# eburhansjah/ec504_ImageEncoder

Hardware: AMD Instinct MI355X
Metric: 1080p I-frames/s (higher is better)
Workload: dtype f32 (colour fast path, FDCT: exact integers in floats) + f64 (colour ties) + int32 (VLC, packing); 1 GPU; 300 x 1920x1080 synthetic RGB frames per GPU, FULL region (all macroblocks), quality_factor 12, input and output resident in HBM; frames_per_gpu=300, global_frames=300, parallelism=frames sharded 300/GPU

## Files before the change

### ec504_imageencoder_amd/csrc/m1v_encode_tile_body.h

```cpp
    extern __shared__ __attribute__((aligned(16))) uint32_t lds[];
    const Geometry &g = a.g;
    const int tid = threadIdx.x;
    const int lane = tid & (kWave - 1);
    const int wave = __builtin_amdgcn_readfirstlane(tid >> 6);
    const bool chroma = wave == 2;
    constexpr int kStride = STAGE8 ? kStageStride8 : kStageStride16;

    uint32_t *vlc = lds + kTileVlc + wave * kVlcWords, *cnt = lds + kTileCnt, *G = lds + kTileG, *segtab = lds + kTileSegTab, *misc = lds + kTileMisc;
    const uint32_t lds0 = (uint32_t)(uintptr_t)(__attribute__((address_space(3))) uint32_t *)lds;
    const uint32_t region_off = (uint32_t)kTileFixedWords * 4u + (uint32_t)wave * a.luma_region;
    uint32_t *image = lds + kTileFixedWords + (2u * a.luma_region + a.chroma_region) / 4u;

    int frame, tile;
    frame_unit_of(blockIdx.x, a.n_frames, a.div_group, a.div_frame, frame, tile);
    const int tk = (int)udiv((uint32_t)tile, a.div_cols), tc = tile - tk * a.tile_cols;
    const int tr = (int)a.tile_row_order[tk];
    tile = tr * a.tile_cols + tc;
    int s0 = tc * kTileStrips, m0 = tr * kTileMbRows;
    const uint8_t *fbase;
    if constexpr (SURFACE) fbase = a.rgb + (unsigned long long)frame * frame_stride;
    else fbase = pixel_stage_rounds_down(a.rgb + (unsigned long long)frame * g.frame_bytes, s0, m0);
    const unsigned long long tile_index = (unsigned long long)frame * a.tiles_per_frame + tile;

    auto owner = [&](int ln, int &j, int &m, int &blk) {
        if (!chroma) {
            m = 2 * wave + (ln >> 5);
            blk = ((ln >> 4) & 1) * 2 + (ln & 1);
            j = (ln >> 1) & 7;
        } else {
            m = (ln >> 3) & 3;
            blk = 4 + (ln >> 5);
            j = ln & 7;
        }
    };
    const int strips_here = min(kTileStrips, g.n_strips - s0);
    int comp;
    {
        int j_, m_, blk_;
        owner(lane, j_, m_, blk_);
        comp = blk_ < 4 ? 0 : blk_ - 3;
    }

    TSTAMP_INIT();
    const uint32_t ring = lds0 + region_off;
    constexpr int kKeep = STAGE8 ? M1V_TILE_KEEP : M1V_TILE_KEEP_WIDE;
    RowStore<kKeep> rows;
    M1V_FRONT_HALF<R, kKeep, !SURFACE, BPP, SURFACE, ORDER>(
        g, fbase, ring, wave, lane, s0, m0, strips_here, comp,
        [&]() {
#pragma unroll
            for (int q = 0; q < kVlcWords / kWave; q++)
                dma4((uint32_t)lane * 4u, lds0 + (uint32_t)(kTileVlc + wave * kVlcWords + q * kWave) * 4u, a.tab->vlc + q * kWave);
        },
        [&]() {
            uint4 *image4 = reinterpret_cast<uint4 *>(image);
            for (int k = tid; k < (a.lds_words >> 2); k += kTileThreads) image4[k] = make_uint4(0u, 0u, 0u, 0u);
        },
        rows, row_pitch);
    const M1V_CONST_AS float *rq_t = reinterpret_cast<const M1V_CONST_AS float *>(reinterpret_cast<uintptr_t>(frame_rq_t(a.rq_all, a.qsel, frame)));
    int j, m, blk;
    {
        int ln = lane;
        asm volatile("" : "+v"(ln));
        owner(ln, j, m, blk);
    }
    const bool valid = j < strips_here && m0 + m < g.n_mbrows;
    const int e = j * kTileSegBlocks + m * 6 + blk;
    uint32_t *blkp = lds + region_off / 4u + lane * kStride;
    uint32_t lds_addr = (uint32_t)(uintptr_t)(__attribute__((address_space(3))) uint32_t *)blkp;
    TSTAMP(2);
    const int dc = columns_to_stage<STAGE8, kKeep>(rows, rq_t, lds_addr);
    const unsigned long long nz = (stage_nonzero_mask<STAGE8>(blkp, lds_addr) & ~1ull) | (dc != 0 ? 1ull : 0ull);
    TSTAMP(3);

    auto fetch = [&](int p) -> int { return fetch_level<STAGE8>(blkp, p); };
    uint32_t hdr = 0, bad = 0;
    int hlen = 0;
    BlockBits bb = {0, 0};
    dc_header(dc, blk < 4, blk, vlc, hdr, hlen);
    const unsigned long long emit = emit_set(nz);
    block_bits_pass1<STAGE8>(hdr, hlen, dc != 0, emit, vlc, fetch, bb.acc, bb.tot, bad);
    if (!valid) {
        bb.tot = 0;
        bad = 0;
    }
    cnt[e] = (uint32_t)bb.tot;
    TSTAMP(4);
    lds_barrier();
    TSTAMP(5);

    const uint32_t c0 = cnt[lane], c1 = cnt[64 + lane], c2 = cnt[128 + lane];
    const uint32_t i0 = wave_scan_inclusive(c0), i1 = wave_scan_inclusive(c1), i2 = wave_scan_inclusive(c2);
    const uint32_t t0 = (uint32_t)__builtin_amdgcn_readlane((int)i0, 63), t1 = (uint32_t)__builtin_amdgcn_readlane((int)i1, 63);
    G[lane] = i0 - c0;
    G[64 + lane] = t0 + i1 - c1;
    G[128 + lane] = t0 + t1 + i2 - c2;
    if (lane == 63) G[192] = t0 + t1 + i2;
    const uint32_t slice_bits = tr == 0 ? 38u : 0u;
    const uint32_t gs = G[min(lane, 8) * kTileSegBlocks];
    const uint32_t gs_next = (uint32_t)__builtin_amdgcn_update_dpp(0, (int)gs, 0x101, 0xf, 0xf, true);
    const uint32_t seg_bits = lane < strips_here ? slice_bits + (gs_next - gs) : 0u;
    const uint32_t seg_words = lane < 8 ? (seg_bits + 31u) >> 5 : 0u;
    const uint32_t seg_incl = row_scan_inclusive(seg_words);
    const uint32_t end_words = (uint32_t)__builtin_amdgcn_readlane((int)seg_incl, 7);
    if (lane < 8) {
        segtab[2 * lane] = gs;
        segtab[2 * lane + 1] = seg_incl - seg_words;
    }
    const uint32_t my_gs = segtab[2 * j], my_base = segtab[2 * j + 1];
    const uint32_t off = my_base * 32u + slice_bits + (G[e] - my_gs);
    TSTAMP(6);

    auto walk = [&](auto &sink) { walk_codes<STAGE8>(hdr, hlen, dc != 0, emit, vlc, fetch, sink); };
    unsigned long long *const strip_ctr_s0 = a.strip_ctr + ((unsigned long long)frame * (unsigned)g.n_strips + (unsigned)s0);
    auto strip_arrives = [&](uint32_t bits) -> unsigned long long {
#ifdef M1V_TILE_NOCOMPLETE
        __hip_atomic_fetch_add(strip_ctr_s0 + lane, (1ull << kCtrCountShift) | (unsigned long long)bits,
                               __ATOMIC_RELAXED, __HIP_MEMORY_SCOPE_AGENT);
        return 0ull;
#endif
        return atomicAdd(strip_ctr_s0 + lane, (1ull << kCtrCountShift) | (unsigned long long)bits);
    };
    auto strip_completes = [&](unsigned long long before, uint32_t bits) {
        if ((uint32_t)(before >> kCtrCountShift) == (uint32_t)a.tile_rows - 1u)
            atomicAdd(&a.frame_bytes[frame], ((before & kCtrBitsMask) + bits + 7ull) >> 3);
    };
    uint2 *seg_out = a.seg + (((unsigned long long)frame * (unsigned)a.tile_rows + (unsigned)tr) * (unsigned)g.n_strips + (unsigned)s0) + lane;
    auto slice_headers = [&](uint32_t *img, bool swapped) {
        if (tr == 0) {
            const uint32_t h0 = slice_word0(s0 + lane), h1 = kSliceWord1, w = seg_incl - seg_words;
            atomicOr(&img[w], swapped ? __builtin_bswap32(h0) : h0);
            atomicOr(&img[w + 1], swapped ? __builtin_bswap32(h1) : h1);
        }
    };

    if (end_words + 2 > (uint32_t)a.lds_words) {
        if (tid == 0) misc[0] = atomicAdd(a.arena_next, 1u);
        __syncthreads();
        const uint32_t got = misc[0];
        if (got >= a.arena_slots) {
            if (tid == 0) atomicOr(a.status, (uint32_t)M1V_STATUS_SCRATCH);
            if (wave == 0 && lane < strips_here) {
                *seg_out = make_uint2(0u, 0u);
                strip_completes(strip_arrives(0u), 0u);
            }
            return;
        }
        const unsigned long long where = a.arena_off + (unsigned long long)got * a.run_cap;
        uint32_t *big = reinterpret_cast<uint32_t *>(a.scratch + where);
        for (uint32_t i = tid; i < (a.run_cap >> 2); i += kTileThreads) big[i] = 0;
        __syncthreads();
        if (wave == 0 && lane < strips_here) {
            slice_headers(big, true);
            *seg_out = make_uint2(seg_bits, (uint32_t)(where >> 2) + (seg_incl - seg_words));
            strip_completes(strip_arrives(seg_bits), seg_bits);
        }
        if (valid) put_block<true>(big, off, bb, walk);
        if (bad) atomicOr(a.status, (uint32_t)M1V_STATUS_UNENCODABLE);
        return;
    }

    unsigned long long arrived = 0;
    if (wave == 0 && lane < strips_here) {
        slice_headers(image, false);
        *seg_out = make_uint2(seg_bits, (uint32_t)((tile_index * a.slot_bytes) >> 2) + (seg_incl - seg_words));
        arrived = strip_arrives(seg_bits);
    }
    if (valid) put_block<false>(image, off, bb, walk);
    TSTAMP(7);
    lds_barrier();
    TSTAMP(8);
    if (wave == 0 && lane < strips_here) strip_completes(arrived, seg_bits);
    uint32_t *slot32 = reinterpret_cast<uint32_t *>(a.scratch + tile_index * a.slot_bytes);
    for (uint32_t i = tid; i < end_words; i += kTileThreads) slot32[i] = __builtin_bswap32(image[i]);
    if (bad) atomicOr(a.status, (uint32_t)M1V_STATUS_UNENCODABLE);
    TSTAMP(9);
    TSTAMP_FLUSH();
```

### ec504_imageencoder_amd/csrc/m1v_kernels.hip

```cpp
#include <hip/hip_runtime.h>

#include <math.h>
#include <stdint.h>
#include <stdio.h>
#include <stdlib.h>
#include <string.h>

#include <type_traits>
#include <algorithm>
#include <vector>

#include "../../include/mpeg1_hip.h"

#define M1V_HD __host__ __device__ __forceinline__
#include "fdct_f32.h"

#pragma clang fp contract(off)

namespace {

constexpr int kWave = 64;
constexpr int kAcRows = 32;
constexpr int kVlcRowInfo = 0, kVlcEntries = 32, kVlcDcLuma = 144, kVlcDcChroma = 160, kVlcWords = 192;
constexpr int kMaxBlockBits = 886;
constexpr int kDefaultLdsWords = 4096;

__host__ __device__ constexpr int scan_pos(int k) {
    constexpr int t[64] = {0,  1,  5,  6,  14, 15, 27, 28, 2,  4,  7,  13, 16, 26, 29, 42,
                           3,  8,  12, 17, 25, 30, 41, 43, 9,  11, 18, 24, 31, 40, 44, 53,
                           10, 19, 23, 32, 39, 45, 52, 54, 20, 22, 33, 38, 46, 51, 55, 60,
                           21, 34, 37, 47, 50, 56, 59, 61, 35, 36, 48, 49, 57, 58, 62, 63};
    return t[k];
}
__host__ __device__ constexpr int scan_inv(int p) {
    for (int k = 0; k < 64; k++)
        if (scan_pos(k) == p) return k;
    return -1;
}

constexpr int kStageStride8 = 17, kStageStride16 = 33;
__host__ __device__ constexpr int stage_byte8(int p) { return ((p & 7) + 8 * (p >> 5)) * 4 + ((p >> 3) & 3); }
__host__ __device__ constexpr int stage_byte16(int p) { return ((p & 15) + 16 * (p >> 5)) * 4 + 2 * ((p >> 4) & 1); }

struct Tables {
    float rq[64];
    float rq_t[64];
    uint32_t vlc[kVlcWords];
    uint8_t hdr[256][44];
};

struct Geometry {
    int W, H, C;
    int n_strips, n_mbrows;
    int half_w;
    uint32_t strip_cap;
    unsigned long long frame_bytes;
};

#ifdef M1V_STAMPS
#define STAMP(ph)                                                                                  \
    do {                                                                                           \
        __builtin_amdgcn_sched_barrier(0);                                                         \
        unsigned long long now_ = __builtin_amdgcn_s_memtime();                                    \
        __builtin_amdgcn_s_waitcnt(0xC07F);                                                        \
        if ((threadIdx.x & 63) == 0) atomicAdd(&a.stamps[ph], now_ - stamp_t_);                    \
        stamp_t_ = __builtin_amdgcn_s_memtime();                                                   \
        __builtin_amdgcn_s_waitcnt(0xC07F);                                                        \
        __builtin_amdgcn_sched_barrier(0);                                                         \
    } while (0)
#define STAMP_INIT() unsigned long long stamp_t_ = __builtin_amdgcn_s_memtime(); __builtin_amdgcn_s_waitcnt(0xC07F)
#elif defined(M1V_MARKS)
#define STAMP(ph) asm volatile("; PHASE_MARK " #ph ::: "memory")
#define STAMP_INIT() asm volatile("; PHASE_MARK start" ::: "memory")
#else
#define STAMP(ph) do { } while (0)
#define STAMP_INIT() do { } while (0)
#endif

struct EncodeArgs {
    Geometry g;
    const uint8_t *rgb;
    const Tables *tab;
    const float *rq_all;
    const uint32_t *qsel;
    uint8_t *scratch;
    uint2 *seg;
    unsigned long long *strip_ctr;
    unsigned long long *frame_bytes;
    uint32_t *status;
    int n_frames;
    int threads;
    int lds_words;
    unsigned long long *stamps;
};


__device__ __forceinline__ int component_fp64(int r, int g, int b, double k0, double kr, double kg,
                                              double kb) {
    double acc = k0 + kr * (double)r;
    acc = acc + kg * (double)g;
    acc = acc + kb * (double)b;
    return (int)acc;
}

struct CompCoef {
    double k0, kr, kg, kb;
};
__device__ __forceinline__ CompCoef comp_coef(int comp) {
    CompCoef c;
    c.k0 = comp == 0 ? 0.0 : 128.0;
    c.kr = comp == 0 ? 0.299 : (comp == 1 ? -0.168736 : 0.5);
    c.kg = comp == 0 ? 0.587 : (comp == 1 ? -0.331264 : -0.418688);
    c.kb = comp == 0 ? 0.114 : (comp == 1 ? 0.5 : -0.081312);
    return c;
}

constexpr float kEps = 1.5e-4f;
struct CompCoefF {
    float k0, kr, kg, kb;
    CompCoef d;
};
__device__ __forceinline__ CompCoefF comp_coef_f(int comp) {
    CompCoefF c;
    c.k0 = (comp == 0 ? 0.0f : 128.0f) + 256.0f + kEps;
    c.kr = comp == 0 ? 0.299f : (comp == 1 ? -0.168736f : 0.5f);
    c.kg = comp == 0 ? 0.587f : (comp == 1 ? -0.331264f : -0.418688f);
    c.kb = comp == 0 ? 0.114f : (comp == 1 ? 0.5f : -0.081312f);
    c.d = comp_coef(comp);
    return c;
}
__device__ __forceinline__ CompCoefF comp_coef_wave(bool luma_wave, int lane) {
    CompCoefF c;
    if (luma_wave) {
        asm volatile("");
        c = comp_coef_f(0);
    } else {
        asm volatile("");
        const CompCoefF cb = comp_coef_f(1), cr = comp_coef_f(2);
        const bool hi = lane >= 32;
        c.k0 = cb.k0;
        c.kr = hi ? cr.kr : cb.kr;
        c.kg = hi ? cr.kg : cb.kg;
        c.kb = hi ? cr.kb : cb.kb;
        c.d.k0 = cb.d.k0;
        c.d.kr = hi ? cr.d.kr : cb.d.kr;
        c.d.kg = hi ? cr.d.kg : cb.d.kg;
        c.d.kb = hi ? cr.d.kb : cb.d.kb;
    }
    return c;
}

constexpr float kFracLow = 10.0f / 32768.0f;
__device__ __forceinline__ float component_t(uint32_t r, uint32_t g, uint32_t b, const CompCoefF &k) {
    float t = fmaf((float)b, k.kb, k.k0);
    t = fmaf((float)g, k.kg, t);
    return fmaf((float)r, k.kr, t);
}
__device__ __forceinline__ float clear_fraction(float t) { return __uint_as_float(__float_as_uint(t) & 0xffff8000u); }
__device__ __forceinline__ float component_raw(uint32_t r, uint32_t g, uint32_t b, const CompCoefF &k) {
    const float t = component_t(r, g, b, k);
    float p = clear_fraction(t);
    if (t - p < kFracLow) {
        const CompCoef &d = k.d;
        p = m1vf::kPxBiasF + (float)component_fp64((int)r, (int)g, (int)b, d.k0, d.kr, d.kg, d.kb);
    }
    return p;
}

#define M1V_CONST_AS __attribute__((address_space(4)))

__device__ __forceinline__ const float *frame_rq_t(const float *rq_all, const uint32_t *qsel, int frame) {
    const M1V_CONST_AS uint32_t *sel = reinterpret_cast<const M1V_CONST_AS uint32_t *>(reinterpret_cast<uintptr_t>(qsel));
    return rq_all + sel[frame];
}


__device__ __forceinline__ const uint8_t *pixel_stage_rounds_down(const uint8_t *frame_base, int &u0, int &u1) {
    unsigned long long p = (unsigned long long)(uintptr_t)frame_base;
    asm volatile("s_setreg_imm32_b32 hwreg(HW_REG_MODE, 0, 2), 2" : "+s"(p), "+s"(u0), "+s"(u1));
    return (const uint8_t *)(uintptr_t)p;
}

struct __attribute__((aligned(4))) Row24 {
    uint32_t d[6];
};

template <int BPP, bool LEAN, int ORDER = 0, typename RowT>
__device__ __forceinline__ void convert_row(const RowT &v, const CompCoefF &k, float out[8]) {
    auto chan = [&](int j, int ch) -> uint32_t {
        int byte = BPP * j + (ORDER ? 2 - ch : ch);
        return (v.d[byte >> 2] >> ((byte & 3) * 8)) & 0xffu;
    };
    float lowest = 1.0f;
#pragma unroll
    for (int j = 0; j < 8; j += 2) {
        const float t0 = component_t(chan(j, 0), chan(j, 1), chan(j, 2), k);
        const float t1 = component_t(chan(j + 1, 0), chan(j + 1, 1), chan(j + 1, 2), k);
        out[j] = clear_fraction(t0);
        out[j + 1] = clear_fraction(t1);
        lowest = fminf(fminf(lowest, t0 - out[j]), t1 - out[j + 1]);
    }
    if (lowest < kFracLow) {
        RowT w = v;
        if constexpr (LEAN) {
#pragma unroll
            for (int i = 0; i < (int)(sizeof(RowT) / 4); i++) asm("" : "+v"(w.d[i]));
        }
        auto chan2 = [&](int j, int ch) -> uint32_t {
            int byte = BPP * j + (ORDER ? 2 - ch : ch);
            return (w.d[byte >> 2] >> ((byte & 3) * 8)) & 0xffu;
        };
        const CompCoef &d = k.d;
#pragma unroll
        for (int j = 0; j < 8; j++) {
            const uint32_t r = chan2(j, 0), gg = chan2(j, 1), b = chan2(j, 2);
            const float t = component_t(r, gg, b, k);
            if (t - clear_fraction(t) < kFracLow)
                out[j] = m1vf::kPxBiasF + (float)component_fp64((int)r, (int)gg, (int)b, d.k0, d.kr, d.kg, d.kb);
        }
    }
}

template <bool FAST>
__device__ __forceinline__ void load_row(const uint8_t *p, int C, const CompCoefF &k, float out[8]) {
    if (FAST) {
        Row24 v = *reinterpret_cast<const Row24 *>(p);
        convert_row<3, false>(v, k, out);
    } else {
#pragma unroll
        for (int j = 0; j < 8; j++) {
            const uint8_t *q = p + j * C;
            out[j] = component_raw(q[0], q[1], q[2], k);
        }
    }
}


__device__ __forceinline__ int quant(float n, float rq) { return (int)(n * rq); }

struct BlockSrc {
    uint32_t first;
    uint32_t stride;
    int blk;
    __device__ int comp() const { return blk < 4 ? 0 : blk - 3; }
};
__device__ __forceinline__ BlockSrc block_source(const Geometry &g, int strip, int bidx) {
    BlockSrc s;
    int mb = bidx / 6;
    s.blk = bidx - mb * 6;
    if (s.blk < 4) {
        int x0 = strip * 16 + (s.blk & 1) * 8;
        int y0 = mb * 16 + (s.blk >> 1) * 8;
        s.first = (uint32_t)y0 * (uint32_t)g.W + (uint32_t)x0;
        s.stride = (uint32_t)g.W;
    } else {
        s.first = (uint32_t)(mb * 8) * (uint32_t)g.half_w + (uint32_t)(strip * 8);
        s.stride = (uint32_t)g.half_w;
    }
    return s;
}


template <bool FAST>
__device__ __forceinline__ void block_coefficients(const Geometry &g, const uint8_t *frame,
                                                   const BlockSrc &s, const float *rq, int q[64]) {
    float rows[64];
    CompCoefF k = comp_coef_f(s.comp());
#pragma unroll
    for (int i = 0; i < 8; i++) {
        float px[8];
        load_row<FAST>(frame + (size_t)((s.first + (uint32_t)i * s.stride) * (uint32_t)g.C), g.C, k, px);
        m1vf::fdct_row_f<float, false>(px, &rows[i * 8]);
    }
#pragma unroll
    for (int i = 0; i < 8; i++) {
        float c[8];
        m1vf::fdct_col_f<float>(rows[0 * 8 + i], rows[1 * 8 + i], rows[2 * 8 + i], rows[3 * 8 + i], rows[4 * 8 + i],
                                rows[5 * 8 + i], rows[6 * 8 + i], rows[7 * 8 + i], c, i == 0 ? 8.0f * m1vf::kPxBiasF : 0.0f);
#pragma unroll
        for (int u = 0; u < 8; u++) q[u * 8 + i] = quant(c[u], rq[u * 8 + i]);
    }
}


template <bool NARROW>
__device__ __forceinline__ void ac_code(const uint32_t *vlc, int r, int level, uint32_t &code, uint32_t &bits, uint32_t &bad) {
    const uint32_t L = (uint32_t)(level < 0 ? -level : level);
    const uint32_t info = vlc[kVlcRowInfo + min(r, kAcRows - 1)];
    const bool in_table = r < kAcRows && L - 1u < (info >> 8);
    const uint32_t e = vlc[kVlcEntries + (in_table ? (info & 0xffu) + L - 1u : 0u)];
    const uint32_t head = (1u << 6) | ((uint32_t)r & 0x3fu);
    const uint32_t lo = (uint32_t)level & 0xffu;
    uint32_t esc = (head << 8) | lo, esc_bits = 20;
    if (!NARROW) {
        const bool wide = L >= 128u;
        esc = wide ? (head << 16) | (level < 0 ? 0x8000u : 0u) | lo : esc;
        esc_bits = wide ? 28 : 20;
        bad |= (!in_table && L >= 256u) ? 1u : 0u;
    }
    code = in_table ? (e & 0xffffu) : esc;
    bits = in_table ? (e >> 16) : esc_bits;
}

template <bool NARROW, typename Fetch>
__device__ __forceinline__ void block_bits_pass1(uint32_t hdr, int hlen, bool dc_nonzero, unsigned long long emit,
                                                 const uint32_t *vlc, Fetch fetch, unsigned long long &acc, int &tot,
                                                 uint32_t &bad) {
    acc = hdr;
    tot = hlen;
    int prev = dc_nonzero ? 0 : -1;
    while (emit) {
// ... 1674 lines not shown
```

### ec504_imageencoder_amd/csrc/m1v_size_table_body.h

```cpp
    extern __shared__ __attribute__((aligned(16))) uint32_t lds[];
    const Geometry &g = a.g;
    const int tid = threadIdx.x;
    const int lane = tid & (kWave - 1);
    const int wave = __builtin_amdgcn_readfirstlane(tid >> 6);
    const bool chroma = wave == 2;
    constexpr int kStride = STAGE8 ? kStageStride8 : kStageStride16;
    const uint32_t *vlc = lds + wave * kVlcWords;
    uint32_t *cnt = lds + kTableCnt;
    [[maybe_unused]] uint32_t *rd_part = lds + kTableFixedWords + 3u * (a.region / 4u);
    const uint32_t lds0 = (uint32_t)(uintptr_t)(__attribute__((address_space(3))) uint32_t *)lds;
    const uint32_t region_off = (uint32_t)kTableFixedWords * 4u + (uint32_t)wave * a.region;

    int frame, tile;
    frame_unit_of(blockIdx.x, a.n_frames, a.div_group, a.div_frame, frame, tile);
    const int tk = (int)udiv((uint32_t)tile, a.div_cols), tc = tile - tk * a.tile_cols;
    const int tr = (int)a.tile_row_order[tk];
    const int s0 = tc * kTileStrips, m0 = tr * kTileMbRows;
    const uint8_t *fbase = a.rgb + (unsigned long long)frame * (SURFACE ? frame_stride : g.frame_bytes);
    auto owner = [&](int ln, int &j, int &m, int &blk) {
        if (!chroma) {
            m = 2 * wave + (ln >> 5);
            blk = ((ln >> 4) & 1) * 2 + (ln & 1);
            j = (ln >> 1) & 7;
        } else {
            m = (ln >> 3) & 3;
            blk = 4 + (ln >> 5);
            j = ln & 7;
        }
    };
    const int strips_here = min(kTileStrips, g.n_strips - s0);
    int comp;
    {
        int j_, m_, blk_;
        owner(lane, j_, m_, blk_);
        comp = blk_ < 4 ? 0 : blk_ - 3;
    }

    RowStore<8> rows;
    M1V_FRONT_HALF<R, 8, false, BPP, SURFACE, ORDER>(
        g, fbase, lds0 + region_off, wave, lane, s0, m0, strips_here, comp,
        [&]() {
#pragma unroll
            for (int q = 0; q < kVlcWords / kWave; q++)
                dma4((uint32_t)lane * 4u, lds0 + (uint32_t)(wave * kVlcWords + q * kWave) * 4u, a.tab->vlc + q * kWave);
        },
        [] {}, rows, row_pitch);
    float coef[64];
#pragma unroll
    for (int i = 0; i < 8; i++) {
        float c[8];
        m1vf::fdct_col_f<float>(rows.get(0, i), rows.get(1, i), rows.get(2, i), rows.get(3, i), rows.get(4, i), rows.get(5, i),
                                rows.get(6, i), rows.get(7, i), c, i == 0 ? RowStore<8>::kBias0 : 0.0f);
#pragma unroll
        for (int u = 0; u < 8; u++) coef[u * 8 + i] = c[u];
    }
    [[maybe_unused]] float sumsq = 0.0f;
    if constexpr (RD) {
#pragma unroll
        for (int t = 0; t < 64; t++) sumsq = __builtin_fmaf(coef[t], coef[t], sumsq);
    }
    int j, m, blk;
    {
        int ln = lane;
        asm volatile("" : "+v"(ln));
        owner(ln, j, m, blk);
    }
    const bool valid = j < strips_here && m0 + m < g.n_mbrows;
    const int e = j * kTileSegBlocks + m * 6 + blk;
    const uint32_t *blkp = lds + region_off / 4u + lane * kStride;
    auto fetch = [&](int p) -> int { return fetch_level<STAGE8>(blkp, p); };

    uint32_t bad_q = 0;
    for (int k = 0; k < a.n_q; k++) {
        const M1V_CONST_AS float *rq_t = reinterpret_cast<const M1V_CONST_AS float *>(reinterpret_cast<uintptr_t>(a.rq_all + a.qoff[k]));
        uint32_t lds_addr = (uint32_t)(uintptr_t)(__attribute__((address_space(3))) const uint32_t *)blkp;
        asm volatile("" : "+v"(lds_addr) : : "memory");
        int dc = 0;
#pragma unroll
        for (int i = 0; i < 8; i++) {
#pragma unroll
            for (int u = 0; u < 8; u++) {
                const int q = quant(coef[u * 8 + i], rq_t[i * 8 + u]);
                const int p = scan_pos(u * 8 + i);
                if (p == 0) dc = q;
                if (STAGE8)
                    asm("ds_write_b8 %0, %1 offset:%2" : "+v"(lds_addr) : "v"(q), "n"(stage_byte8(p)));
                else
                    asm("ds_write_b16 %0, %1 offset:%2" : "+v"(lds_addr) : "v"(q), "n"(stage_byte16(p)));
            }
        }
        const unsigned long long nz = (stage_nonzero_mask<STAGE8>(blkp, lds_addr) & ~1ull) | (dc != 0 ? 1ull : 0ull);
        uint32_t hdr = 0, bad = 0;
        int hlen = 0;
        BlockBits bb = {0, 0};
        dc_header(dc, blk < 4, blk, vlc, hdr, hlen);
        block_bits_pass1<STAGE8>(hdr, hlen, dc != 0, emit_set(nz), vlc, fetch, bb.acc, bb.tot, bad);
        cnt[k * kTileThreads + e] = valid ? (uint32_t)bb.tot : 0u;
        bad_q |= (valid && bad) ? 1u << k : 0u;
        if constexpr (RD) {
            const M1V_CONST_AS float *dq_t = reinterpret_cast<const M1V_CONST_AS float *>(reinterpret_cast<uintptr_t>(rd_dq + a.qoff[k]));
            const unsigned long long keep = emit_set(nz) | 1ull;
            const uint32_t keep_lo = (uint32_t)keep, keep_hi = (uint32_t)(keep >> 32);
            float gain = 0.0f;
#pragma unroll
            for (int i = 0; i < 8; i++) {
#pragma unroll
                for (int u = 0; u < 8; u++) {
                    const int p = scan_pos(u * 8 + i);
                    const float c = coef[u * 8 + i];
                    const float t = __builtin_truncf(c * rq_t[i * 8 + u]) * dq_t[i * 8 + u];
                    const float w = __builtin_fmaf(2.0f, c, -t);
                    const int carried = (int)((p < 32 ? keep_lo : keep_hi) << (31 - (p & 31))) >> 31;
                    gain = __builtin_fmaf(__uint_as_float(__float_as_uint(t) & (uint32_t)carried), w, gain);
                }
            }
            const uint32_t dw = wave_sum_u32(valid ? (uint32_t)(sumsq - gain) : 0u);
            if (lane == 0) rd_part[k * 3 + wave] = dw;
        }
    }
    lds_barrier();

    if (wave == 0) {
        const int k = lane >> 3, jj = lane & 7;
        if (k < a.n_q && jj < strips_here) {
            const uint4 *c4 = reinterpret_cast<const uint4 *>(cnt + k * kTileThreads + jj * kTileSegBlocks);
            uint32_t bits = tr == 0 ? 38u : 0u;
#pragma unroll
            for (int t = 0; t < kTileSegBlocks / 4; t++) {
                const uint4 v = c4[t];
                bits += v.x + v.y + v.z + v.w;
            }
            const unsigned long long kf = (unsigned long long)k * (unsigned)a.n_frames + (unsigned)frame;
            const unsigned long long before = atomicAdd(a.strip_ctr + kf * (unsigned)g.n_strips + (unsigned)(s0 + jj),
                                                        (1ull << kCtrCountShift) | (unsigned long long)bits);
            if ((uint32_t)(before >> kCtrCountShift) == (uint32_t)a.tile_rows - 1u)
                atomicAdd(&a.frame_bytes[kf], ((before & kCtrBitsMask) + bits + 7ull) >> 3);
            if constexpr (RD)
                if (jj == 0) atomicAdd(rd_dist + kf, (unsigned long long)rd_part[k * 3] + rd_part[k * 3 + 1] + rd_part[k * 3 + 2]);
        }
    }
    for (uint32_t b = bad_q; b; b &= b - 1u) atomicOr(&a.status[__builtin_ctz(b)], (uint32_t)M1V_STATUS_UNENCODABLE);
```

### ec504_imageencoder_amd/csrc/m1v_tiles.h

```cpp

constexpr int kTileStrips = 8, kTileMbRows = 4;
constexpr int kTileThreads = kTileStrips * kTileMbRows * 6;
constexpr int kTileSegBlocks = kTileMbRows * 6;
constexpr int kTileSlot = 2048;
constexpr int kTileVlc = 0, kTileCnt = 3 * kVlcWords, kTileG = kTileCnt + 192, kTileSegTab = kTileG + 196, kTileMisc = kTileSegTab + 16,
              kTileFixedWords = kTileMisc + 4;

struct TileArgs {
    Geometry g;
    const uint8_t *rgb;
    const Tables *tab;
    const float *rq_all;
    const uint32_t *qsel;
    uint8_t *scratch;
    uint2 *seg;
    unsigned long long *strip_ctr;
    unsigned long long *frame_bytes;
    uint32_t *arena_next;
    uint32_t slot_bytes, arena_slots;
    unsigned long long arena_off;
    uint32_t *status;
    int n_frames;
    int tile_cols, tile_rows, tiles_per_frame;
    DivMagic div_group, div_frame, div_cols;
    const uint32_t *tile_row_order;
    int lds_words;
    uint32_t run_cap;
    uint32_t luma_region, chroma_region;
    unsigned long long *stamps;
};

__device__ __forceinline__ void dma16(uint32_t voff, uint32_t ldsdst, const uint8_t *sbase) {
    uint32_t keep;
    asm volatile("s_mov_b32 %0, m0\n\ts_mov_b32 m0, %2\n\ts_nop 0\n\tglobal_load_lds_dwordx4 %1, %3\n\ts_mov_b32 m0, %0"
                 : "=&s"(keep)
                 : "v"(voff), "s"(ldsdst), "s"(sbase));
}
__device__ __forceinline__ void dma4(uint32_t voff, uint32_t ldsdst, const void *sbase) {
    uint32_t keep;
    asm volatile("s_mov_b32 %0, m0\n\ts_mov_b32 m0, %2\n\ts_nop 0\n\tglobal_load_lds_dword %1, %3\n\ts_mov_b32 m0, %0"
                 : "=&s"(keep)
                 : "v"(voff), "s"(ldsdst), "s"(sbase));
}
template <int N>
__device__ __forceinline__ void wait_vm() {
    asm volatile("s_waitcnt vmcnt(%0)" ::"n"(N));
}
__device__ __forceinline__ void lds_barrier() { asm volatile("s_waitcnt lgkmcnt(0)\n\ts_barrier" ::: "memory"); }

__device__ __forceinline__ Row24 ring_read24(uint32_t addr) {
    unsigned long long r0, r1, r2;
    asm volatile("ds_read_b64 %0, %3\n\tds_read_b64 %1, %3 offset:8\n\tds_read_b64 %2, %3 offset:16\n\ts_waitcnt lgkmcnt(0)"
                 : "=&v"(r0), "=&v"(r1), "=&v"(r2)
                 : "v"(addr));
    Row24 v;
    v.d[0] = (uint32_t)r0; v.d[1] = (uint32_t)(r0 >> 32);
    v.d[2] = (uint32_t)r1; v.d[3] = (uint32_t)(r1 >> 32);
    v.d[4] = (uint32_t)r2; v.d[5] = (uint32_t)(r2 >> 32);
    return v;
}

__device__ __forceinline__ Row32 ring_read32(uint32_t addr) {
    typedef uint32_t u32x4 __attribute__((ext_vector_type(4)));
    u32x4 r0, r1;
    asm volatile("ds_read_b128 %0, %2\n\tds_read_b128 %1, %2 offset:16\n\ts_waitcnt lgkmcnt(0)"
                 : "=&v"(r0), "=&v"(r1)
                 : "v"(addr));
    Row32 v;
    v.d[0] = r0.x; v.d[1] = r0.y; v.d[2] = r0.z; v.d[3] = r0.w;
    v.d[4] = r1.x; v.d[5] = r1.y; v.d[6] = r1.z; v.d[7] = r1.w;
    return v;
}

template <bool STAGE8, int KEEP>
__device__ __forceinline__ int columns_to_stage(const RowStore<KEEP> &rows, const M1V_CONST_AS float *rq_t, uint32_t &lds_addr) {
    int dc = 0;
#pragma unroll
    for (int i = 0; i < 8; i++) {
        float c[8];
        m1vf::fdct_col_f<float>(rows.get(0, i), rows.get(1, i), rows.get(2, i), rows.get(3, i), rows.get(4, i), rows.get(5, i),
                                rows.get(6, i), rows.get(7, i), c, i == 0 ? RowStore<KEEP>::kBias0 : 0.0f);
#pragma unroll
        for (int u = 0; u < 8; u++) {
            const int q = quant(c[u], rq_t[i * 8 + u]);
            const int p = scan_pos(u * 8 + i);
            if (p == 0) dc = q;
            if (STAGE8)
                asm("ds_write_b8 %0, %1 offset:%2" : "+v"(lds_addr) : "v"(q), "n"(stage_byte8(p)));
            else
                asm("ds_write_b16 %0, %1 offset:%2" : "+v"(lds_addr) : "v"(q), "n"(stage_byte16(p)));
        }
    }
    return dc;
}

#ifndef M1V_TILE_KEEP
#define M1V_TILE_KEEP 8
#endif
#ifndef M1V_TILE_KEEP_WIDE
#define M1V_TILE_KEEP_WIDE 2
#endif
#ifdef M1V_TILE_STAMPS
#define TSTAMP(ph)                                                                                 \
    do {                                                                                           \
        __builtin_amdgcn_sched_barrier(0);                                                         \
        const unsigned long long now_ = __builtin_amdgcn_s_memtime();                              \
        asm volatile("s_waitcnt lgkmcnt(0)");                                                      \
        tstamp_[ph] += now_ - tstamp_t_;                                                           \
        tstamp_t_ = now_;                                                                          \
        __builtin_amdgcn_sched_barrier(0);                                                         \
    } while (0)
#define TSTAMP_INIT()                                                                              \
    unsigned long long tstamp_[12] = {0, 0, 0, 0, 0, 0, 0, 0, 0, 0, 0, 0};                          \
    unsigned long long tstamp_t_ = __builtin_amdgcn_s_memtime();                                   \
    asm volatile("s_waitcnt lgkmcnt(0)")
#define TSTAMP_FLUSH()                                                                             \
    do {                                                                                           \
        if (lane == 0)                                                                             \
            for (int ph_ = 0; ph_ < 12; ph_++) atomicAdd(&a.stamps[ph_ + (chroma ? 12 : 0)], tstamp_[ph_]); \
    } while (0)
#else
#define TSTAMP(ph) do { } while (0)
#define TSTAMP_INIT() do { } while (0)
#define TSTAMP_FLUSH() do { } while (0)
#endif

#ifndef M1V_TILE_LEAN
#define M1V_TILE_LEAN false
#endif
#define M1V_PACKED_INPUT                                                                           \
    constexpr bool SURFACE = false;                                                                \
    constexpr int ORDER = 0;                                                                       \
    constexpr uint32_t row_pitch = 0;                                                              \
    constexpr unsigned long long frame_stride = 0
#define M1V_FRONT_HALF tile_pixel_rows
#ifndef M1V_TILE_WAVES_PER_EU
#define M1V_TILE_WAVES_PER_EU 5
#endif

template <int R, int KEEP, bool DOWN = true, int BPP = 3, bool SURFACE = false, int ORDER = 0, typename First, typename Meanwhile>
__device__ __forceinline__ void tile_pixel_rows(const Geometry &g, const uint8_t *fbase, uint32_t ring, int wave, int lane, int s0,
                                                int m0, int strips_here, int comp, First first, Meanwhile meanwhile,
                                                RowStore<KEEP> &rows, uint32_t row_pitch = 0) {
    const bool chroma = wave == 2;
    uint32_t pitch;
    uint32_t voff_a, voff_b;
    uint32_t lane_row;
    const uint32_t third = (uint32_t)(lane >= 24) + (uint32_t)(lane >= 48);
    auto uniform = [](uint32_t v) {
        asm volatile("" : "+s"(v));
        return v;
    };
    if constexpr (BPP == 4) {
        const uint32_t piece = (uint32_t)lane >> (chroma ? 4 : 5);
        const uint32_t row_px = chroma ? (uint32_t)g.half_w : (uint32_t)g.W;
        pitch = row_px * 4u;
        const uint32_t vw = (uint32_t)strips_here * (chroma ? 32u : 64u);
        const uint32_t within = min(((uint32_t)lane & (chroma ? 15u : 31u)) * 16u, vw - 16u);
        auto row_off = [&](uint32_t pc) {
            if (!chroma) {
                const uint32_t mb = (uint32_t)min(m0 + 2 * wave + (int)(pc >> 1), g.n_mbrows - 1);
                if constexpr (SURFACE) return (mb * 16u + (pc & 1u) * 8u) * row_pitch + (uint32_t)s0 * 64u;
                return ((mb * 16u + (pc & 1u) * 8u) * row_px + (uint32_t)s0 * 16u) * 4u;
            }
            const uint32_t mb = (uint32_t)min(m0 + (int)pc, g.n_mbrows - 1);
            if constexpr (SURFACE) return (mb * 4u) * row_pitch + (uint32_t)s0 * 32u;
            return ((mb * 8u) * row_px + (uint32_t)s0 * 8u) * 4u;
        };
        const uint32_t r0 = uniform(row_off(0)), r1 = uniform(row_off(1)), r2 = uniform(row_off(2)), r3 = uniform(row_off(3));
        if (!chroma) {
            voff_a = (piece ? r1 : r0) + within;
            voff_b = (piece ? r3 : r2) + within;
            lane_row = ring + ((uint32_t)lane << 5);
        } else {
            voff_a = voff_b = (piece == 0 ? r0 : (piece == 1 ? r1 : (piece == 2 ? r2 : r3))) + within;
            lane_row = ring + (((uint32_t)lane & 31u) << 5);
        }
    } else if (!chroma) {
        pitch = (uint32_t)g.W * 3u;
        const uint32_t vw = (uint32_t)strips_here * 48u;
        auto row_off = [&](uint32_t piece) {
            const uint32_t mb = (uint32_t)min(m0 + 2 * wave + (int)(piece >> 1), g.n_mbrows - 1);
            if constexpr (SURFACE) return (mb * 16u + (piece & 1u) * 8u) * row_pitch + (uint32_t)s0 * 48u;
            return ((mb * 16u + (piece & 1u) * 8u) * (uint32_t)g.W + (uint32_t)s0 * 16u) * 3u;
        };
        const uint32_t r0 = uniform(row_off(0)), r1 = uniform(row_off(1)), r2 = uniform(row_off(2)), r3 = uniform(row_off(3));
        voff_a = (third == 0 ? r0 : (third == 1 ? r1 : r2)) + min(((uint32_t)lane - (third << 4) - (third << 3)) * 16u, vw - 16u);
        const uint32_t l5 = (uint32_t)lane & 31u;
        voff_b = l5 < 8u ? r2 + min((16u + l5) * 16u, vw - 16u) : r3 + min((l5 - 8u) * 16u, vw - 16u);
        lane_row = ring + ((uint32_t)lane << 4) + ((uint32_t)lane << 3);
    } else {
        pitch = (uint32_t)g.half_w * 3u;
        const uint32_t vw = (uint32_t)strips_here * 24u;
        const uint32_t L = (uint32_t)lane - (third << 4) - (third << 3), piece = (uint32_t)(L >= 12u), within = min((L - (piece << 3) - (piece << 2)) * 16u, ((vw + 15u) & ~15u) - 16u);
        auto row_off = [&](uint32_t mbrow) {
            const uint32_t mb = (uint32_t)min(m0 + (int)mbrow, g.n_mbrows - 1);
            if constexpr (SURFACE) return (mb * 4u) * row_pitch + (uint32_t)s0 * 24u;
            return ((mb * 8u) * (uint32_t)g.half_w + (uint32_t)s0 * 8u) * 3u;
        };
        const uint32_t r0 = uniform(row_off(0)), r1 = uniform(row_off(1)), r2 = uniform(row_off(2)), r3 = uniform(row_off(3));
        voff_a = (piece ? r1 : r0) + within;
        voff_b = (piece ? r3 : r2) + within;
        const uint32_t mrow = ((uint32_t)lane >> 3) & 3u, l3 = (uint32_t)lane & 7u;
        lane_row = ring + (mrow >> 1) * 1024u + (mrow & 1u) * 192u + (l3 << 4) + (l3 << 3);
    }
    constexpr uint32_t kSlot = 2048;
    const uint32_t step2 = chroma ? row_pitch : 2u * row_pitch, step1 = chroma ? (uint32_t)g.half_w * (uint32_t)BPP : row_pitch;
    auto issue_row = [&](int r) {
        const uint8_t *sb = SURFACE ? fbase + ((size_t)(r >> 1) * step2 + (size_t)(r & 1) * step1) : fbase + (size_t)r * pitch;
        const uint32_t dst = ring + (uint32_t)(r % R) * kSlot;
        uint32_t keep;
        asm volatile("s_mov_b32 %0, m0\n\ts_mov_b32 m0, %3\n\ts_nop 0\n\t"
                     "global_load_lds_dwordx4 %1, %4\n\tglobal_load_lds_dwordx4 %2, %5 offset:1024\n\t"
                     "s_mov_b32 m0, %0"
                     : "=&s"(keep)
                     : "v"(voff_a), "v"(voff_b), "s"(dst), "s"(sb), "s"(sb - 1024));
    };

    first();
#pragma unroll
    for (int r = 0; r < R; r++) issue_row(r);
    meanwhile();

    (void)comp;
    const CompCoefF kf = comp_coef_wave(!chroma, lane);
#pragma unroll
    for (int i = 0; i < 8; i++) {
        const int newest = (i - 1 + R < 7) ? (i - 1 + R) : 7;
        const int behind = newest - i;
        if (behind == 0) wait_vm<0>(); else if (behind == 1) wait_vm<2>(); else if (behind == 2) wait_vm<4>();
        else if (behind == 3) wait_vm<6>(); else if (behind == 4) wait_vm<8>(); else if (behind == 5) wait_vm<10>();
        else if (behind == 6) wait_vm<12>(); else wait_vm<14>();
        float px[8];
        if constexpr (BPP == 4) {
            const Row32 v = ring_read32(lane_row + (uint32_t)(i % R) * kSlot);
            if (i + R < 8) issue_row(i + R);
            convert_row<4, true, ORDER>(v, kf, px);
        } else {
            const Row24 v = ring_read24(lane_row + (uint32_t)(i % R) * kSlot);
            if (i + R < 8) issue_row(i + R);
            convert_row<3, M1V_TILE_LEAN, ORDER>(v, kf, px);
        }
        float ro[8];
        m1vf::fdct_row_f<float, DOWN>(px, ro);
        rows.put(i, ro);
    }
}


template <bool STAGE8, int R>
__global__ __launch_bounds__(kTileThreads) __attribute__((amdgpu_waves_per_eu(M1V_TILE_WAVES_PER_EU, M1V_TILE_WAVES_PER_EU)))
void k_encode_tiles(TileArgs a) {
    constexpr int BPP = 3;
    M1V_PACKED_INPUT;
#include "m1v_encode_tile_body.h"
}

struct SurfaceArgs {
    TileArgs t;
    unsigned long long frame_stride;
    uint32_t row_pitch;
};
template <bool STAGE8, int R, int BPP, int ORDER>
__global__ __launch_bounds__(kTileThreads) __attribute__((amdgpu_waves_per_eu(M1V_TILE_WAVES_PER_EU, M1V_TILE_WAVES_PER_EU)))
void k_encode_surface(SurfaceArgs sa) {
    constexpr bool SURFACE = true;
    const TileArgs &a = sa.t;
    const uint32_t row_pitch = sa.row_pitch;
    const unsigned long long frame_stride = sa.frame_stride;
#include "m1v_encode_tile_body.h"
}

struct CoefTileArgs {
    Geometry g;
    const uint8_t *rgb;
    const Tables *tab;
    int16_t *out;
    int n_frames, tile_cols, tile_rows, tiles_per_frame;
    uint32_t region;
};
constexpr int kCoefStride = 34;

template <int R>
__global__ __launch_bounds__(kTileThreads) __attribute__((amdgpu_waves_per_eu(M1V_TILE_WAVES_PER_EU, M1V_TILE_WAVES_PER_EU)))
void k_coefficient_tiles(CoefTileArgs a) {
    extern __shared__ __attribute__((aligned(16))) uint32_t lds[];
    const Geometry &g = a.g;
    const int tid = threadIdx.x;
    const int lane = tid & (kWave - 1);
    const int wave = __builtin_amdgcn_readfirstlane(tid >> 6);
    const uint32_t lds0 = (uint32_t)(uintptr_t)(__attribute__((address_space(3))) uint32_t *)lds;
    int frame, tile;
    frame_strip_of(blockIdx.x, a.n_frames, a.tiles_per_frame, frame, tile);
    const int tr = tile / a.tile_cols, tc = tile - tr * a.tile_cols;
    int s0 = tc * kTileStrips, m0 = tr * kTileMbRows;
    const uint8_t *fbase = pixel_stage_rounds_down(a.rgb + (unsigned long long)frame * g.frame_bytes, s0, m0);
    const int strips_here = min(kTileStrips, g.n_strips - s0), mrows_here = min(kTileMbRows, g.n_mbrows - m0);
    const int comp = wave == 2 ? 1 + (lane >> 5) : 0;

    RowStore<M1V_TILE_KEEP> rows;
    tile_pixel_rows<R, M1V_TILE_KEEP>(g, fbase, lds0 + (uint32_t)wave * a.region, wave, lane, s0, m0, strips_here, comp, [] {}, [] {}, rows);

    const M1V_CONST_AS float *rq_t = reinterpret_cast<const M1V_CONST_AS float *>(reinterpret_cast<uintptr_t>(a.tab->rq_t));
    uint32_t lds_addr = lds0 + (uint32_t)wave * a.region + (uint32_t)lane * (kCoefStride * 4u);
#pragma unroll
    for (int i = 0; i < 8; i++) {
        float c[8];
        m1vf::fdct_col_f<float>(rows.get(0, i), rows.get(1, i), rows.get(2, i), rows.get(3, i), rows.get(4, i), rows.get(5, i),
                                rows.get(6, i), rows.get(7, i), c, i == 0 ? RowStore<M1V_TILE_KEEP>::kBias0 : 0.0f);
#pragma unroll
        for (int u = 0; u < 8; u++) {
            const int q = quant(c[u], rq_t[i * 8 + u]);
            asm("ds_write_b16 %0, %1 offset:%2" : "+v"(lds_addr) : "v"(q), "n"(2 * scan_pos(u * 8 + i)));
        }
    }
    asm volatile("s_waitcnt lgkmcnt(0)\n\ts_barrier" ::"v"(lds_addr) : "memory");

    const int bps = g.n_mbrows * 6;
    const unsigned char *lds_bytes = reinterpret_cast<const unsigned char *>(lds);
    const int units_valid = mrows_here * 6 * 8;
#pragma unroll
    for (int t = 0; t < kTileStrips * kTileSegBlocks * 8 / kTileThreads; t++) {
        const int u = tid + t * kTileThreads;
        const int j = u / (kTileSegBlocks * 8), within = u - j * (kTileSegBlocks * 8);
        if (j >= strips_here || within >= units_valid) continue;
        const int b = within >> 3, part = within & 7, m = b / 6, blk = b - m * 6;
        const int w_src = blk < 4 ? (m >> 1) : 2;
        const int l_src = blk < 4 ? (m & 1) * 32 + (blk >> 1) * 16 + j * 2 + (blk & 1) : (blk - 4) * 32 + m * 8 + j;
        const unsigned char *from = lds_bytes + (size_t)w_src * a.region + (size_t)l_src * (kCoefStride * 4) + part * 16;
        const uint2 lo = *reinterpret_cast<const uint2 *>(from), hi = *reinterpret_cast<const uint2 *>(from + 8);
        int16_t *o = a.out + (((size_t)frame * g.n_strips + (size_t)(s0 + j)) * bps + (size_t)m0 * 6) * 64;
        *reinterpret_cast<uint4 *>(reinterpret_cast<unsigned char *>(o) + (size_t)within * 16) = make_uint4(lo.x, lo.y, hi.x, hi.y);
    }
}


struct TableArgs {
    Geometry g;
    const uint8_t *rgb;
    const Tables *tab;
    const float *rq_all;
    uint32_t qoff[kMaxCandidates];
    int n_q;
    unsigned long long *strip_ctr;
    unsigned long long *frame_bytes;
    uint32_t *status;
    int n_frames, tile_cols, tile_rows, tiles_per_frame;
    DivMagic div_group, div_frame, div_cols;
    const uint32_t *tile_row_order;
    uint32_t region;
};
constexpr int kTableCnt = 3 * kVlcWords, kTableFixedWords = kTableCnt + kMaxCandidates * kTileThreads;

#define M1V_SIZES_ONLY                                                                             \
    constexpr bool RD = false;                                                                     \
    constexpr const float *rd_dq = nullptr;                                                        \
    constexpr unsigned long long *rd_dist = nullptr

template <bool STAGE8, int R>
__global__ __launch_bounds__(kTileThreads) void k_size_table_tiles(TableArgs a) {
    constexpr int BPP = 3;
    M1V_PACKED_INPUT;
    M1V_SIZES_ONLY;
#include "m1v_size_table_body.h"
}
template <bool STAGE8, int R>
__global__ __launch_bounds__(kTileThreads) void k_size_table_rgba(TableArgs a) {
    constexpr int BPP = 4;
    M1V_PACKED_INPUT;
    M1V_SIZES_ONLY;
#include "m1v_size_table_body.h"
}
struct SurfaceTableArgs {
    TableArgs t;
    unsigned long long frame_stride;
    uint32_t row_pitch;
};
template <bool STAGE8, int R, int BPP, int ORDER>
__global__ __launch_bounds__(kTileThreads) void k_size_table_surface(SurfaceTableArgs sa) {
    constexpr bool SURFACE = true;
    const TableArgs &a = sa.t;
    const uint32_t row_pitch = sa.row_pitch;
    const unsigned long long frame_stride = sa.frame_stride;
    M1V_SIZES_ONLY;
#include "m1v_size_table_body.h"
}

struct TableSizesArgs {
    int n_frames, n_strips;
    unsigned long long *strip_ctr, *frame_bytes;
    uint32_t *status;
    unsigned long long *out_sizes;
    unsigned long long stride;
    uint32_t *out_status;
};
// ... 74 lines not shown
```

Before: 503,300 frames/s.

## Pack quantized levels in registers and store with paired dword writes

Replaces the per-coefficient byte and halfword LDS writes after quantization with packing into registers via SDWA converts, then writes whole words with ds_write2_b32 once each word is complete. The nonzero mask is now built from the packed registers instead of being read back from LDS. The three count reads are also merged into one read plus one paired read. This cuts LDS instruction count and the read-back pass, at the cost of more VGPRs and hand-written inline assembly that depends on the scan-order layout.

```diff
diff --git a/ec504_imageencoder_amd/csrc/m1v_encode_tile_body.h b/ec504_imageencoder_amd/csrc/m1v_encode_tile_body.h
--- a/ec504_imageencoder_amd/csrc/m1v_encode_tile_body.h
+++ b/ec504_imageencoder_amd/csrc/m1v_encode_tile_body.h
@@ -58,6 +58,13 @@
         },
         rows, row_pitch);
     const M1V_CONST_AS float *rq_t = reinterpret_cast<const M1V_CONST_AS float *>(reinterpret_cast<uintptr_t>(frame_rq_t(a.rq_all, a.qsel, frame)));
+    uint32_t *blkp = lds + region_off / 4u + lane * kStride;
+    uint32_t lds_addr = (uint32_t)(uintptr_t)(__attribute__((address_space(3))) uint32_t *)blkp;
+    TSTAMP(2);
+    unsigned long long nz_ac;
+    const int dc = columns_to_stage<STAGE8, kKeep>(rows, rq_t, lds_addr, nz_ac);
+    const unsigned long long nz = nz_ac | (dc != 0 ? 1ull : 0ull);
+    TSTAMP(3);
     int j, m, blk;
     {
         int ln = lane;
@@ -66,12 +73,6 @@
     }
     const bool valid = j < strips_here && m0 + m < g.n_mbrows;
     const int e = j * kTileSegBlocks + m * 6 + blk;
-    uint32_t *blkp = lds + region_off / 4u + lane * kStride;
-    uint32_t lds_addr = (uint32_t)(uintptr_t)(__attribute__((address_space(3))) uint32_t *)blkp;
-    TSTAMP(2);
-    const int dc = columns_to_stage<STAGE8, kKeep>(rows, rq_t, lds_addr);
-    const unsigned long long nz = (stage_nonzero_mask<STAGE8>(blkp, lds_addr) & ~1ull) | (dc != 0 ? 1ull : 0ull);
-    TSTAMP(3);
 
     auto fetch = [&](int p) -> int { return fetch_level<STAGE8>(blkp, p); };
     uint32_t hdr = 0, bad = 0;
@@ -89,7 +90,12 @@
     lds_barrier();
     TSTAMP(5);
 
-    const uint32_t c0 = cnt[lane], c1 = cnt[64 + lane], c2 = cnt[128 + lane];
+    uint32_t c0;
+    unsigned long long c12;
+    asm volatile("ds_read_b32 %0, %2\n\tds_read2_b32 %1, %2 offset0:64 offset1:128\n\ts_waitcnt lgkmcnt(0)"
+                 : "=&v"(c0), "=&v"(c12)
+                 : "v"(lds0 + (uint32_t)(kTileCnt + lane) * 4u));
+    const uint32_t c1 = (uint32_t)c12, c2 = (uint32_t)(c12 >> 32);
     const uint32_t i0 = wave_scan_inclusive(c0), i1 = wave_scan_inclusive(c1), i2 = wave_scan_inclusive(c2);
     const uint32_t t0 = (uint32_t)__builtin_amdgcn_readlane((int)i0, 63), t1 = (uint32_t)__builtin_amdgcn_readlane((int)i1, 63);
     G[lane] = i0 - c0;
diff --git a/ec504_imageencoder_amd/csrc/m1v_kernels.hip b/ec504_imageencoder_amd/csrc/m1v_kernels.hip
--- a/ec504_imageencoder_amd/csrc/m1v_kernels.hip
+++ b/ec504_imageencoder_amd/csrc/m1v_kernels.hip
@@ -7,6 +7,7 @@
 #include <string.h>
 
 #include <type_traits>
+#include <utility>
 #include <algorithm>
 #include <vector>
 
diff --git a/ec504_imageencoder_amd/csrc/m1v_size_table_body.h b/ec504_imageencoder_amd/csrc/m1v_size_table_body.h
--- a/ec504_imageencoder_amd/csrc/m1v_size_table_body.h
+++ b/ec504_imageencoder_amd/csrc/m1v_size_table_body.h
@@ -76,20 +76,13 @@
         uint32_t lds_addr = (uint32_t)(uintptr_t)(__attribute__((address_space(3))) const uint32_t *)blkp;
         asm volatile("" : "+v"(lds_addr) : : "memory");
         int dc = 0;
-#pragma unroll
-        for (int i = 0; i < 8; i++) {
-#pragma unroll
-            for (int u = 0; u < 8; u++) {
-                const int q = quant(coef[u * 8 + i], rq_t[i * 8 + u]);
-                const int p = scan_pos(u * 8 + i);
-                if (p == 0) dc = q;
-                if (STAGE8)
-                    asm("ds_write_b8 %0, %1 offset:%2" : "+v"(lds_addr) : "v"(q), "n"(stage_byte8(p)));
-                else
-                    asm("ds_write_b16 %0, %1 offset:%2" : "+v"(lds_addr) : "v"(q), "n"(stage_byte16(p)));
-            }
-        }
-        const unsigned long long nz = (stage_nonzero_mask<STAGE8>(blkp, lds_addr) & ~1ull) | (dc != 0 ? 1ull : 0ull);
+        StagePack<STAGE8> pk;
+        static_for<64>([&](auto N) {
+            constexpr int n = decltype(N)::value, i = n >> 3, u = n & 7;
+            dc |= pk.template level<n>(coef[u * 8 + i], rq_t[i * 8 + u], lds_addr);
+        });
+        pk.finish(lds_addr);
+        const unsigned long long nz = pk.mask_and_fence(lds_addr) | (dc != 0 ? 1ull : 0ull);
         uint32_t hdr = 0, bad = 0;
         int hlen = 0;
         BlockBits bb = {0, 0};
diff --git a/ec504_imageencoder_amd/csrc/m1v_tiles.h b/ec504_imageencoder_amd/csrc/m1v_tiles.h
--- a/ec504_imageencoder_amd/csrc/m1v_tiles.h
+++ b/ec504_imageencoder_amd/csrc/m1v_tiles.h
@@ -72,25 +72,139 @@
     return v;
 }
 
+template <int... Is, typename F>
+__device__ __forceinline__ void static_for_each(std::integer_sequence<int, Is...>, F &&f) { (f(std::integral_constant<int, Is>{}), ...); }
+template <int N, typename F>
+__device__ __forceinline__ void static_for(F &&f) { static_for_each(std::make_integer_sequence<int, N>{}, f); }
+
+template <bool STAGE8>
+struct StagePack {
+    static constexpr int kWords = STAGE8 ? 16 : 32, kParts = STAGE8 ? 4 : 2;
+    static constexpr int pos(int n) { return scan_pos((n & 7) * 8 + (n >> 3)); }
+    static constexpr int word(int n) { return (STAGE8 ? stage_byte8(pos(n)) : stage_byte16(pos(n))) >> 2; }
+    static constexpr int part(int n) { return STAGE8 ? (stage_byte8(pos(n)) & 3) : ((stage_byte16(pos(n)) >> 1) & 1); }
+    static constexpr bool first(int n) {
+        for (int k = 1; k < n; k++)
+            if (word(k) == word(n)) return false;
+        return true;
+    }
+    static constexpr int done(int w) {
+        int last = 0;
+        for (int n = 1; n < 64; n++)
+            if (word(n) == w) last = n;
+        return last >> 3;
+    }
+    static constexpr int pair(int col, int k, int which) {
+        int held = -1;
+        for (int c = 0; c < 8; c++) {
+            int seen = 0;
+            for (int w = 0; w < kWords; w++) {
+                if (done(w) != c) continue;
+                if (held < 0) {
+                    held = w;
+                    continue;
+                }
+                if (c == col && seen == k) return which ? w : held;
+                seen++;
+                held = -1;
+            }
+        }
+        return -1;
+    }
+
+    uint32_t w[kWords];
+    float t;
+
+    template <int N, bool LAST = false>
+    __device__ __forceinline__ void convert(float c_next, float rq_next) {
+        constexpr int W = word(N), P = part(N);
+        if constexpr (LAST) {
+            if constexpr (STAGE8)
+                asm("v_cvt_i32_f32_sdwa %0, %1 dst_sel:BYTE_%2 dst_unused:UNUSED_PRESERVE src0_sel:DWORD\n\ts_nop 0" : "+v"(w[W]) : "v"(t), "n"(P));
+            else
+                asm("v_cvt_i32_f32_sdwa %0, %1 dst_sel:WORD_%2 dst_unused:UNUSED_PRESERVE src0_sel:DWORD\n\ts_nop 0" : "+v"(w[W]) : "v"(t), "n"(P));
+        } else if constexpr (first(N)) {
+            if constexpr (STAGE8)
+                asm("v_cvt_i32_f32_sdwa %0, %2 dst_sel:BYTE_%5 dst_unused:UNUSED_PAD src0_sel:DWORD\n\tv_mul_f32 %1, %4, %3"
+                    : "=&v"(w[W]), "=v"(t) : "v"(t), "v"(c_next), "s"(rq_next), "n"(P));
+            else
+                asm("v_cvt_i32_f32_sdwa %0, %2 dst_sel:WORD_%5 dst_unused:UNUSED_PAD src0_sel:DWORD\n\tv_mul_f32 %1, %4, %3"
+                    : "=&v"(w[W]), "=v"(t) : "v"(t), "v"(c_next), "s"(rq_next), "n"(P));
+        } else {
+            if constexpr (STAGE8)
+                asm("v_cvt_i32_f32_sdwa %0, %2 dst_sel:BYTE_%5 dst_unused:UNUSED_PRESERVE src0_sel:DWORD\n\tv_mul_f32 %1, %4, %3"
+                    : "+v"(w[W]), "=v"(t) : "v"(t), "v"(c_next), "s"(rq_next), "n"(P));
+            else
+                asm("v_cvt_i32_f32_sdwa %0, %2 dst_sel:WORD_%5 dst_unused:UNUSED_PRESERVE src0_sel:DWORD\n\tv_mul_f32 %1, %4, %3"
+                    : "+v"(w[W]), "=v"(t) : "v"(t), "v"(c_next), "s"(rq_next), "n"(P));
+        }
+    }
+    template <int N>
+    __device__ __forceinline__ int level(float c, float rq, uint32_t &lds_addr) {
+        if constexpr (N == 0) {
+            return quant(c, rq);
+        } else if constexpr (N == 1) {
+            t = c * rq;
+            return 0;
+        } else {
+            convert<N - 1>(c, rq);
+            if constexpr ((N & 7) == 0) store<(N >> 3) - 1>(lds_addr);
+            return 0;
+        }
+    }
+    __device__ __forceinline__ void finish(uint32_t &lds_addr) {
+        convert<63, true>(0.0f, 0.0f);
+        store<7>(lds_addr);
+    }
+    template <int COL, int K = 0>
+    __device__ __forceinline__ void store(uint32_t &lds_addr) {
+        constexpr int A = pair(COL, K, 0), B = pair(COL, K, 1);
+        if constexpr (A >= 0) {
+            asm("ds_write2_b32 %0, %1, %2 offset0:%3 offset1:%4" : "+v"(lds_addr) : "v"(w[A]), "v"(w[B]), "n"(A), "n"(B));
+            store<COL, K + 1>(lds_addr);
+        }
+    }
+    __device__ __forceinline__ unsigned long long mask_and_fence(uint32_t &lds_addr) const {
+        uint32_t half[2] = {0u, 0u};
+#pragma unroll
+        for (int h = 0; h < 2; h++) {
+            if (STAGE8) {
+#pragma unroll
+                for (int j = 0; j < 8; j++) {
+                    const uint32_t f = ((w[h * 8 + j] & 0x7f7f7f7fu) + 0x7f7f7f7fu) | w[h * 8 + j];
+                    half[h] |= (f >> (7 - j)) & (0x01010101u << j);
+                }
+            } else {
+#pragma unroll
+                for (int j = 0; j < 16; j++) {
+                    const uint32_t f = ((w[h * 16 + j] & 0x7fff7fffu) + 0x7fff7fffu) | w[h * 16 + j];
+                    half[h] |= (f >> (15 - j)) & (0x00010001u << j);
+                }
+            }
+        }
+        asm volatile("s_waitcnt lgkmcnt(0)" : "+v"(half[0]), "+v"(half[1]), "+v"(lds_addr) : : "memory");
+        return ((unsigned long long)half[1] << 32) | half[0];
+    }
+};
+static_assert(StagePack<true>::pair(3, 0, 0) == -1 && StagePack<true>::pair(4, 0, 0) == 0 && StagePack<true>::pair(4, 0, 1) == 1, "narrow staging plan");
+
 template <bool STAGE8, int KEEP>
-__device__ __forceinline__ int columns_to_stage(const RowStore<KEEP> &rows, const M1V_CONST_AS float *rq_t, uint32_t &lds_addr) {
+__device__ __forceinline__ int columns_to_stage(const RowStore<KEEP> &rows, const M1V_CONST_AS float *rq_t, uint32_t &lds_addr,
+                                                unsigned long long &nz) {
     int dc = 0;
-#pragma unroll
-    for (int i = 0; i < 8; i++) {
+    StagePack<STAGE8> pk;
+    static_for<8>([&](auto I) {
+        constexpr int i = decltype(I)::value;
         float c[8];
         m1vf::fdct_col_f<float>(rows.get(0, i), rows.get(1, i), rows.get(2, i), rows.get(3, i), rows.get(4, i), rows.get(5, i),
                                 rows.get(6, i), rows.get(7, i), c, i == 0 ? RowStore<KEEP>::kBias0 : 0.0f);
-#pragma unroll
-        for (int u = 0; u < 8; u++) {
-            const int q = quant(c[u], rq_t[i * 8 + u]);
-            const int p = scan_pos(u * 8 + i);
-            if (p == 0) dc = q;
-            if (STAGE8)
-                asm("ds_write_b8 %0, %1 offset:%2" : "+v"(lds_addr) : "v"(q), "n"(stage_byte8(p)));
-            else
-                asm("ds_write_b16 %0, %1 offset:%2" : "+v"(lds_addr) : "v"(q), "n"(stage_byte16(p)));
-        }
-    }
+        static_for<8>([&](auto U) {
+            constexpr int u = decltype(U)::value;
+            dc |= pk.template level<i * 8 + u>(c[u], rq_t[i * 8 + u], lds_addr);
+        });
+    });
+    pk.finish(lds_addr);
+    nz = pk.mask_and_fence(lds_addr);
     return dc;
 }
 
```

New measurement: 522,200 frames/s (median of 6 runs). 3.8% higher.
